# crockwell/pixelsynth

Hardware: AMD Instinct MI355X
Metric: novel-view frames/sec @256x256 (reproject+AR outpaint) (higher is better)
Workload: dtype f32

## Files before the change

### pixelsynth_amd/csrc/lmconv_grid.hip

```cpp
#include "lmconv_handle.h"

namespace pslm {

struct GemmTap {
    const float *in;
    const float *w;
    int dr, dc;
    int mask_row;
    int ld;
};

struct ItemMap {
    const int32_t *order;
    int npre;
    const int32_t *start;
    int f0;
    const int32_t *perm;
    const int2 *permq;
    const int32_t *end;
};
__device__ __forceinline__ int item_at(const ItemMap &m, int pos, int nitems)
{
    if (pos >= nitems) return -1;
    return m.perm ? m.perm[pos] : pos;
// ... 539 lines not shown
                    for (int q = 0; q < NBU; ++q) bv[h][q] = bn[h][q];
                if (j < 4) bload(j + 1, bn);
            } else {
                bload(j, bv);
            }
            __builtin_amdgcn_sched_barrier(0);
            CH_STAMP(3 * j);
            if (ALL) {
#pragma unroll
                for (int h = 0; h < NGH; ++h)
#pragma unroll
                    for (int c = 0; c < 4; ++c)
#pragma unroll
                        for (int k = 0; k < NTL; ++k)
                            acc[k] = __builtin_amdgcn_mfma_f32_16x16x4f32(av[h][a_of(k)][c], bv[h][b_of(k)][c], h == 0 && c == 0 ? zero : acc[k], 0, 0, 0);
#pragma unroll
                for (int k = 0; k < NTL; ++k) taptot[k] = j == 0 ? acc[k] : taptot[k] + acc[k];
            } else {
#pragma unroll
                for (int k = 0; k < NTL; ++k) {
                    if (!lv[k]) continue;
#pragma unroll
                    for (int h = 0; h < NGH; ++h)
#pragma unroll
                        for (int c = 0; c < 4; ++c)
                            acc[k] = __builtin_amdgcn_mfma_f32_16x16x4f32(av[h][a_of(k)][c], bv[h][b_of(k)][c], h == 0 && c == 0 ? zero : acc[k], 0, 0, 0);
                    taptot[k] = j == 0 ? acc[k] : taptot[k] + acc[k];
                }
            }
            CH_STAMP(3 * j + 1);
#pragma unroll
            for (int h = 0; h < NGH; ++h)
#pragma unroll
                for (int n = 0; n < NAU; ++n) av[h][n] = an[h][n];
#ifdef PS_WG_CHAIN_STAMPS
            __builtin_amdgcn_s_waitcnt(0x0F70);
#endif
            CH_STAMP(3 * j + 2);
            __builtin_amdgcn_sched_barrier(0);
        }
        CH_STAMP(15);
#pragma unroll
        for (int k = 0; k < NTL; ++k)
            if (lv[k]) tot[k] = tot[k] + taptot[k];
    };
    auto tap_dispatch = [&](int t, int nxt, int buf) {
        if (has5 && tiles_of(t) == (1u << TI) - 1u) tap_products(t, nxt, buf, std::integral_constant<bool, true>{});
        else tap_products(t, nxt, buf, std::integral_constant<bool, false>{});
    };
#ifndef PS_WG_TAP_SYNCTHREADS
    auto tap_barrier = [] { lds_barrier(); };
#else
    auto tap_barrier = [] { __syncthreads(); };
#endif
    int cur = next_live(-1), buf = 0;
    if (cur < ntaps) {
        stage_load(cur);
        a0_load(cur);
        stage_store(cur, 0);
    }
    __syncthreads();
    WG_STAMP(2);
    int nstamp = 3;
    (void)nstamp;
    for (int slot = 0; slot < a.nslots; ++slot) {
        for (int t = a.slot_first[slot]; t < a.slot_first[slot + 1]; ++t) {
            if (t != cur) continue;
            CH_STAMP(16);
            const int nxt = next_live(t);
            if (nxt < ntaps) stage_load(nxt);
            CH_STAMP(17);
            tap_dispatch(t, nxt, buf);
            CH_STAMP(18);
            if (DB) {
                if (nxt < ntaps) stage_store(nxt, buf ^ 1);
                CH_STAMP(19);
                tap_barrier();
                CH_STAMP(20);
                buf ^= 1;
            } else {
                tap_barrier();
                if (nxt < ntaps) stage_store(nxt, 0);
                tap_barrier();
            }
            cur = nxt;
            WG_STAMP(nstamp < 14 ? nstamp : 13);
#ifdef PS_WG_TRACE_BUILD
            ++tapno;
#endif
            ++nstamp;
        }
        if (slot == SLOT_SKIP) {
            if (fuse_post) {
                float *sY = (float *)sB;
#pragma unroll
                for (int k = 0; k < NTL; ++k)
                    if (k < NT4 || has5) *(f32x4 *)(sY + m_of(k) * YLD + NF + o_of(k) + kk * 4) = tot[k];
            } else {
#pragma unroll
                for (int k = 0; k < NTL; ++k) {
                    const int item = (k < NT4 || has5) ? sItem[m_of(k)] : -1;
                    if (item >= 0) *(f32x4 *)(a.partial + ((size_t)SLOT_SKIP * a.nitems + item) * a.Co_pad + o_of(k) + kk * 4) = tot[k];
                }
            }
        } else {
#pragma unroll
            for (int k = 0; k < NTL; ++k)
                ysum[k] = (slot == SLOT_NA ? *(const f32x4 *)(a.sum_bias + o_of(k) + kk * 4) : ysum[k]) + tot[k];
            if (slot == SLOT_NB && !fuse_post) {
#pragma unroll
                for (int k = 0; k < NTL; ++k) {
                    const int item = (k < NT4 || has5) ? sItem[m_of(k)] : -1;
                    if (item >= 0) *(f32x4 *)(a.partial + ((size_t)SLOT_NA * a.nitems + item) * a.Co_pad + o_of(k) + kk * 4) = ysum[k];
                }
            }
        }
#pragma unroll
        for (int k = 0; k < NTL; ++k) tot[k] = zero;
    }
    WG_STAMP(14);
    if (fuse_post) {
        float *sY = (float *)sB;
        Post4<POSTK, MI / GW_WAVES, GW_WAVES> post;
        post.prefetch(pa, wave, lane, sItem, sLoc);
#pragma unroll
        for (int k = 0; k < NTL; ++k)
            if (k < NT4 || has5) *(f32x4 *)(sY + m_of(k) * YLD + o_of(k) + kk * 4) = ysum[k];
        __syncthreads();
        post.run(pa, lane, sY, YLD);
    }
    WG_STAMP(15);
#ifdef PS_WG_TRACE_BUILD
    __syncthreads();
    if (a.trace_on && (y & 127) == 0 && (y >> 7) < 32 && tid < 96) g_wg_chain[KIND][y >> 7][tid / 24][tid % 24] = sChain[tid / 24][tid % 24];
#endif
    span_end();
}

#ifndef PS_WS_EXP
#define PS_WS_EXP 0
#endif
constexpr int WS_WAVES = 4, WS_THREADS = 64 * WS_WAVES, WS_MI = 16 * WS_WAVES;
constexpr int ws_occ(int kind) { return kind == GW_CONVOUT ? 2 : 3; }
template <int KIND>
__attribute__((amdgpu_waves_per_eu(ws_occ(KIND), ws_occ(KIND))))
__global__ __launch_bounds__(WS_THREADS) void k_gemm_ws(GemmArgs a, PostArgs pa)
{
    constexpr int NGH = KIND == GW_DIL ? 1 : 2, NOT = KIND == GW_CONVOUT ? 10 : 5, CO = 16 * NOT, MI = WS_MI;
    constexpr int POSTK = KIND == GW_CONVOUT ? POST_GATE : KIND == GW_CONVIN ? POST_CONVIN : POST_DIL;
    constexpr int YLD = KIND == GW_DIL ? 84 : 168;
    constexpr int HALF = 4 * CO;
    constexpr int CHUNK = NGH * HALF;
    constexpr int SVN = (CHUNK + WS_THREADS - 1) / WS_THREADS;
    constexpr int NQ = NGH * NOT;
    constexpr int NB4 = 2 * CHUNK > MI * YLD / 4 ? 2 * CHUNK : MI * YLD / 4;
    __shared__ f32x4 sA[NB4];
    __shared__ int sRow[MAX_TAPS * MI];
    __shared__ float sMv[MAX_TAPS * MI];
    __shared__ int sItem[MI], sLoc[MI];
    const int tid = threadIdx.x, wave = __builtin_amdgcn_readfirstlane(tid >> 6), lane = tid & 63, i = lane & 15, kk = lane >> 4;
    const int xcd = blockIdx.x & (N_XCD - 1), tb = blockIdx.x >> 3;
    const int y = xcd * a.tpx + tb;
    if (tb >= a.tpx || y >= a.ny) return;
    const int item0 = y * MI, ntaps = a.slot_first[a.nslots];
    const f32x4 zero = {0.0f, 0.0f, 0.0f, 0.0f};
    {
        const int pos = item0 + lane;
        int item = -1, q = 0, pat = 0x1ff;
        bool frac = true;
        if (pos < a.nitems) {
            if (a.items.permq) {
                const int2 v = a.items.permq[pos];
                item = v.x; q = v.y & 4095; pat = (v.y >> 12) & 0x1ff; frac = (v.y >> 21) & 1;
            } else {
                int fq;
                item = item_at(a.items, pos, a.nitems);
                item_loc(a.items, item, a.L, fq, q);
            }
        }
        const bool valid = item >= 0 && item_wanted(a.items, item);
        const int f = a.items.f0 + (item >= 0 ? item / a.items.npre : 0), r = q / a.W, c = q - r * a.W;
        if (wave == 0) { sItem[lane] = valid ? item : -1; sLoc[lane] = valid ? f * a.L + q : 0; }
        for (int t = wave; t < ntaps; t += WS_WAVES) {
            const GemmTap tp = a.tap[t];
            const int rr = r + tp.dr, cc = c + tp.dc;
            float mv = 0.0f;
            if (valid) {
                if (tp.mask_row < 0) mv = 1.0f;
                else if (!frac) mv = (pat >> tp.mask_row) & 1 ? 1.0f : 0.0f;
                else if (rr >= 0 && rr < a.H && cc >= 0 && cc < a.W) mv = a.mask[(size_t)f * a.mask_fstride + (size_t)tp.mask_row * a.L + q];
            }
            sRow[t * MI + lane] = mv != 0.0f ? (f * a.L + rr * a.W + cc) : -1;
            sMv[t * MI + lane] = mv;
        }
    }
    __syncthreads();
    unsigned wg_live = 0, my_live = 0;
    for (int t = 0; t < ntaps; ++t) {
        const unsigned long long b = __ballot(sRow[t * MI + lane] >= 0);
        if (b) wg_live |= 1u << t;
        if ((b >> (16 * wave)) & 0xFFFFull) my_live |= 1u << t;
    }
    if (wg_live == 0 && __ballot(sItem[lane] >= 0) == 0ull) return;
    auto next_live = [&](int t) {
        int n = t + 1;
        while (n < ntaps && !((wg_live >> n) & 1u)) ++n;
        return n;
    };
    int goff[SVN], loff[SVN];
#pragma unroll
    for (int sx = 0; sx < SVN; ++sx) {
        const int e = min(tid + WS_THREADS * sx, CHUNK - 1), h = e / HALF, r = e - h * HALF, k4 = r / CO, o = r - k4 * CO;
        goff[sx] = h * 5 * HALF + r;
        loff[sx] = h * HALF + (o >> 4) * 64 + k4 * 16 + (o & 15);
    }
    f32x4 sv[SVN];
    auto w_load = [&](int t, int j) {
        const f32x4 *w = (const f32x4 *)a.tap[t].w + j * HALF;
#pragma unroll
        for (int sx = 0; sx < SVN; ++sx) sv[sx] = w[goff[sx]];
    };
    auto w_store = [&](int buf) {
#pragma unroll
        for (int sx = 0; sx < SVN; ++sx)
            if (sx < SVN - 1 || CHUNK % WS_THREADS == 0 || tid + WS_THREADS * sx < CHUNK) sA[buf * CHUNK + loff[sx]] = sv[sx];
    };
    const float *bsrc = nullptr;
    float bmv = 0.0f;
    bool bopen = false;
    f32x4 bn[NGH];
    auto b_tap = [&](int t) {
        const int row = sRow[t * MI + wave * 16 + i];
        bmv = sMv[t * MI + wave * 16 + i];
        bopen = row >= 0;
        bsrc = (bopen ? a.tap[t].in + (size_t)row * a.tap[t].ld : (const float *)g_zero_row) + 4 * kk;
    };
    auto b_load = [&](int j) {
#pragma unroll
        for (int h = 0; h < NGH; ++h) bn[h] = *(const f32x4 *)(bsrc + 16 * (j + 5 * h));
    };
    f32x4 tot[NOT], ysum[NOT];
#pragma unroll
    for (int k = 0; k < NOT; ++k) { tot[k] = zero; ysum[k] = zero; }
    int cur = next_live(-1), buf = 0;
    if (cur < ntaps) {
        w_load(cur, 0);
        b_tap(cur);
        b_load(0);
        w_store(0);
    }
    lds_barrier();
    for (int slot = 0; slot < a.nslots; ++slot) {
        for (int t = a.slot_first[slot]; t < a.slot_first[slot + 1]; ++t) {
            if (t != cur) continue;
            const int nxt = next_live(t);
            const bool mine = (my_live >> t) & 1u;
            f32x4 taptot[NOT];
#pragma unroll
            for (int j = 0; j < 5; ++j) {
                if (!(PS_WS_EXP & 2)) { if (j < 4) w_load(t, j + 1); else w_load(nxt < ntaps ? nxt : t, 0); }
                f32x4 bv[NGH];
#pragma unroll
                for (int h = 0; h < NGH; ++h) bv[h] = bopen ? bn[h] * bmv : zero;
                if (j == 4) b_tap(nxt < ntaps ? nxt : t);
                if (!(PS_WS_EXP & 4)) b_load(j < 4 ? j + 1 : 0);
                if (mine && !(PS_WS_EXP & 1)) {
                    const f32x4 *A = sA + buf * CHUNK + lane;
                    f32x4 acc[NOT], w0 = A[0], w1 = A[64], w2 = zero, w3 = zero;
#pragma unroll
                    for (int q = 0; q < NQ; q += 2) {
                        if (q + 2 < NQ) w2 = A[((q + 2) / NOT) * HALF + ((q + 2) % NOT) * 64];
                        if (q + 3 < NQ) w3 = A[((q + 3) / NOT) * HALF + ((q + 3) % NOT) * 64];
                        __builtin_amdgcn_sched_barrier(0);
                        const int h0 = q / NOT, k0 = q % NOT, h1 = (q + 1) / NOT, k1 = (q + 1) % NOT;
#pragma unroll
                        for (int c = 0; c < 4; ++c) {
                            acc[k0] = __builtin_amdgcn_mfma_f32_16x16x4f32(w0[c], bv[h0][c], h0 == 0 && c == 0 ? zero : acc[k0], 0, 0, 0);
                            if (q + 1 < NQ)
                                acc[k1] = __builtin_amdgcn_mfma_f32_16x16x4f32(w1[c], bv[h1][c], h1 == 0 && c == 0 ? zero : acc[k1], 0, 0, 0);
                        }
                        __builtin_amdgcn_sched_barrier(0);
                        w0 = w2;
                        w1 = w3;
                    }
#pragma unroll
                    for (int k = 0; k < NOT; ++k) taptot[k] = j == 0 ? acc[k] : taptot[k] + acc[k];
                }
                if (!(PS_WS_EXP & 2)) w_store(buf ^ 1);
                if (!(PS_WS_EXP & 8)) lds_barrier();
                buf ^= 1;
            }
            if (mine && !(PS_WS_EXP & 1)) {
#pragma unroll
                for (int k = 0; k < NOT; ++k) tot[k] = tot[k] + taptot[k];
            }
            cur = nxt;
        }
        if (slot == SLOT_SKIP) {
            float *sY = (float *)sA;
#pragma unroll
            for (int k = 0; k < NOT; ++k) *(f32x4 *)(sY + (wave * 16 + i) * YLD + NF + 16 * k + kk * 4) = tot[k];
        } else {
#pragma unroll
            for (int k = 0; k < NOT; ++k) ysum[k] = (slot == SLOT_NA ? *(const f32x4 *)(a.sum_bias + 16 * k + kk * 4) : ysum[k]) + tot[k];
        }
#pragma unroll
        for (int k = 0; k < NOT; ++k) tot[k] = zero;
    }
    {
        float *sY = (float *)sA;
        Post4<POSTK, MI / WS_WAVES, WS_WAVES> post;
        post.prefetch(pa, wave, lane, sItem, sLoc);
#pragma unroll
        for (int k = 0; k < NOT; ++k) *(f32x4 *)(sY + (wave * 16 + i) * YLD + 16 * k + kk * 4) = ysum[k];
        __syncthreads();
        if (!(PS_WS_EXP & 16)) post.run(pa, lane, sY, YLD);
    }
}

struct StartsArgs {
    const int32_t *order;
    const float *mask_und, *mask_dil;
    int H, W, L, npre, F;
    int g_in[NGATED], g_out[NGATED], g_skip[NGATED], d_in[4], d_out[4];
    int32_t *starts;
    int f0;
    const int32_t *pend;
};
constexpr int STARTS_MAXL = 4096;
__global__ __launch_bounds__(1024) void k_prefix_starts(StartsArgs a)
{
    __shared__ int rank[STARTS_MAXL];
    __shared__ int s1[STARTS_MAXL];
    __shared__ int s2[STARTS_MAXL];
    __shared__ int cmin[2];
    const int f = a.f0 + blockIdx.x, t = threadIdx.x, L = a.L, npre = a.pend ? a.pend[f] : a.npre;
    const int32_t *ord = a.order + (size_t)f * L;
    for (int r = t; r < L; r += 1024) rank[ord[r]] = r;
    if (t < 2) cmin[t] = npre;
    __syncthreads();
    for (int r = t; r < L; r += 1024) {
        const int q = ord[r], y = q / a.W, x = q - y * a.W;
        int m1 = npre, m2 = npre;
        for (int tap = 0; tap < 9; ++tap) {
            if (tap == 4) continue;
            const int dy = tap / 3 - 1, dx = tap % 3 - 1;
            if (a.mask_und[((size_t)f * 9 + tap) * L + q] != 0.0f) {
                const int yy = y + dy, xx = x + dx;
                if (yy >= 0 && yy < a.H && xx >= 0 && xx < a.W) m1 = min(m1, rank[yy * a.W + xx]);
            }
            if (a.mask_dil[((size_t)f * 9 + tap) * L + q] != 0.0f) {
                const int yy = y + 2 * dy, xx = x + 2 * dx;
                if (yy >= 0 && yy < a.H && xx >= 0 && xx < a.W) m2 = min(m2, rank[yy * a.W + xx]);
            }
        }
        if (r < npre) { s1[r] = m1; s2[r] = m2; }
        else { atomicMin(&cmin[0], m1); atomicMin(&cmin[1], m2); }
    }
    __syncthreads();
    for (int off = 1; off < npre; off <<= 1) {
        int v1[STARTS_MAXL / 1024], v2[STARTS_MAXL / 1024];
#pragma unroll
        for (int k = 0; k < STARTS_MAXL / 1024; ++k) {
            const int r = t + 1024 * k;
            if (r < npre) {
                v1[k] = r + off < npre ? min(s1[r], s1[r + off]) : s1[r];
                v2[k] = r + off < npre ? min(s2[r], s2[r + off]) : s2[r];
            }
        }
        __syncthreads();
#pragma unroll
        for (int k = 0; k < STARTS_MAXL / 1024; ++k) {
            const int r = t + 1024 * k;
            if (r < npre) { s1[r] = v1[k]; s2[r] = v2[k]; }
        }
        __syncthreads();
    }
    if (t != 0) return;
    auto suf = [&](const int *s, int r0) { return r0 >= npre ? npre : min(r0, s[r0]); };
    int need[NNODE], needX[NGATED];
    for (int n = 0; n < NNODE; ++n) need[n] = npre;
    for (int g = 0; g < NGATED; ++g) { needX[g] = cmin[0]; need[a.g_in[g]] = min(need[a.g_in[g]], cmin[0]); }
    for (int d = 0; d < 4; ++d) need[a.d_in[d]] = min(need[a.d_in[d]], cmin[1]);
    const int kind[18] = {0, 0, 1, 0, 0, 1, 0, 0, 0, 0, 1, 0, 0, 0, 1, 0, 0, 0};
    const int idx[18] = {0, 1, 0, 2, 3, 1, 4, 5, 6, 7, 2, 8, 9, 10, 3, 11, 12, 13};
    int32_t *out = a.starts + f;
    for (int e = 17; e >= 0; --e) {
        if (kind[e] == 0) {
            const int g = idx[e];
            const int so = need[a.g_out[g]];
            out[(size_t)(15 + g) * a.F] = so;
            needX[g] = min(needX[g], suf(s1, so));
            need[a.g_in[g]] = min(need[a.g_in[g]], so);
            const int si = needX[g];
            out[(size_t)(1 + g) * a.F] = si;
            need[a.g_in[g]] = min(need[a.g_in[g]], suf(s1, si));
            if (a.g_skip[g] >= 0) need[a.g_skip[g]] = min(need[a.g_skip[g]], si);
        } else {
            const int d = idx[e];
            const int sd = need[a.d_out[d]];
            out[(size_t)(29 + d) * a.F] = sd;
            need[a.d_in[d]] = min(need[a.d_in[d]], suf(s2, sd));
        }
    }
    out[0] = need[0];
}

struct PermArgs {
    const int32_t *order;
    const float *mask[2];
    int H, W, L, npre, f0, nf, nparts;
    uint32_t *sorted[2];
    int32_t *cnt[2];
    int32_t *tsum[2];
    int32_t *perm[2];
    int2 *permq[2];
    const int32_t *pend;
};
constexpr int PERM_KEYS = 512;
struct PermBins { unsigned short v[PERM_KEYS]; };
constexpr PermBins make_perm_bins()
{
    PermBins t{};
    int n = 0;
    for (int pc = 9; pc >= 0; --pc)
        for (int p = 0; p < PERM_KEYS; ++p)
            if (__builtin_popcount((unsigned)p) == pc) t.v[p] = (unsigned short)n++;
    return t;
}
__device__ const PermBins g_perm_bin = make_perm_bins();
constexpr PermBins make_perm_pats()
{
    PermBins t{}, b = make_perm_bins();
    for (int p = 0; p < PERM_KEYS; ++p) t.v[b.v[p]] = (unsigned short)p;
    return t;
}
__device__ const PermBins g_perm_pat = make_perm_pats();
__device__ __forceinline__ int perm_fpp(const PermArgs &a) { return (a.nf + a.nparts - 1) / a.nparts; }
__device__ __forceinline__ size_t perm_cnt_index(const PermArgs &a, int fl, int key)
{
    const int fpp = perm_fpp(a), part = fl / fpp;
// ... 401 lines not shown
```

### pixelsynth_amd/z_buffermodel.py

```python
import math
import os
import types

import numpy as np
import torch
import torch.nn as nn

from .ar_plan import ARPlan, build_ar_plan, plan_from_reference_args
from .lmconv.layers import PONO
from .lmconv.model import TP_MIN_FRAMES, LaunchPipeline, OurPixelCNN, launch_capacity, wavefronts
from .lmconv.sample import sample
from .networks.f16x3 import checked
from .projection.z_buffer_manipulator import PtsManipulator

_PREFIX_STREAMS = {}


def rank_samples(discrim_scores, entropy_scores):
    n = len(discrim_scores)
    by_disc, by_entr = np.argsort(np.asarray(discrim_scores)), np.argsort(np.asarray(entropy_scores))
    disc_rank, entr_rank = np.empty(n, np.int64), np.empty(n, np.int64)
    disc_rank[by_disc] = np.arange(n)
    entr_rank[by_entr] = np.arange(n)
    return int(np.argmax(.5 * (n - 1 - entr_rank) + .5 * disc_rank))
# ... 25 lines not shown
        self.offset = [torch.tensor([k * V, 0], dtype=torch.int32, device=device) for k in range(depth)]
        self.order[:] = torch.arange(L, device=device, dtype=torch.int32)
        self.args = (self.codes, self.order, self.region, *self.masks)


class ZbufferModelPts(nn.Module):
    def __init__(self, opt, pts_regressor=None, vqvae=None, projector=None, encoder=None, classifier=None):
        super().__init__()
        self.opt = opt
        if pts_regressor is None and hasattr(opt, "norm_G"):
            from .networks import Unet
            extra = {"num_filters": opt.Unet_num_filters} if hasattr(opt, "Unet_num_filters") else {}
            pts_regressor = Unet(channels_in=3, channels_out=1, opt=opt, **extra)
        if projector is None and "resnet" in getattr(opt, "refine_model_type", "") and hasattr(opt, "norm_G"):
            from .networks import get_decoder
            projector = get_decoder(opt)
        self.pts_regressor = pts_regressor
        self.encoder = encoder
        if classifier is None and max(int(getattr(opt, "num_samples", 1)), 1) > 1:
            from .networks import resnet18
            classifier = resnet18(num_classes=365)
        self.classifier = classifier
        if vqvae is None and getattr(opt, "vqvae", False):
            from .vqvae2 import VQVAETop
            vqvae = VQVAETop()
        self.vqvae = vqvae
        self.projector = projector
        C = 3 if getattr(opt, "use_rgb_features", True) else 64
        self.pts_transformer = PtsManipulator(opt.W, C=C, opt=opt)
        self.num_classes = 512
        self.outpaint2 = OurPixelCNN(nr_resnet=2, nr_filters=80, input_channels=self.num_classes,
                                     nr_logistic_mix=10, kernel_size=(3, 3), max_dilation=2, weight_norm=False,
                                     feature_norm_op=lambda c: PONO(), dropout_prob=0, conv_bias=True,
                                     conv_mask_weight=False, rematerialize=False, binarize=False)
        self.args = types.SimpleNamespace(dataloader_seed=getattr(opt, "seed", 0), num_classes=self.num_classes)
        self.obs = [3, 32, 32]
        self.downsample = nn.AvgPool2d(kernel_size=8, stride=8)
        self.rotvecs = {'R': np.array([0, .6, 0]), 'L': np.array([0, -.6, 0]), 'U': np.array([-.3, 0, 0]),
                        'D': np.array([.3, 0, 0]), 'UR': np.array([-.15, .3, 0]), 'UL': np.array([-.15, -.3, 0]),
                        'DR': np.array([.15, .3, 0]), 'DL': np.array([.15, -.3, 0])}
        self.mapping = ['R', 'L', 'U', 'D', 'UL', 'UR', 'DR', 'DL']
        self.sample_batch = 32

    def eulerAnglesToRotationMatrix(self, theta):
        R_x = np.array([[1, 0, 0], [0, math.cos(theta[0]), -math.sin(theta[0])],
                        [0, math.sin(theta[0]), math.cos(theta[0])]])
        R_y = np.array([[math.cos(theta[1]), 0, math.sin(theta[1])], [0, 1, 0],
                        [-math.sin(theta[1]), 0, math.cos(theta[1])]])
        R_z = np.array([[math.cos(theta[2]), -math.sin(theta[2]), 0],
                        [math.sin(theta[2]), math.cos(theta[2]), 0], [0, 0, 1]])
        return np.dot(R_z, np.dot(R_y, R_x))

    def get_rt_from_rot(self, direction, input_RT, num=None, denom=None):
        dev = input_RT.device
        if num is None:
            num = 0
        setting = getattr(self.opt, "model_setting", "gen_img")
        if setting in ('gen_two_imgs', 'gen_scene'):
            if direction == 'S':
                new_RT = torch.zeros_like(input_RT)
                new_RT[:, :, :3] = input_RT[:, :, :3]
                new_RT[:, 3, 3] = 1
                off = torch.tensor([np.sin(2 * np.pi * num / denom), np.cos(2 * np.pi * num / denom),
                                    .4 * np.sin(2 * np.pi * (.25 + num / denom))]).to(dev)
                new_RT[0, :3, 3] = input_RT[0, :3, 3] + .35 * off
                return torch.inverse(new_RT), new_RT
            elif direction == 'C':
                rotvec = np.array([0.2 * np.cos(2 * np.pi * num / denom), 0.2 * np.sin(2 * np.pi * num / denom), 0])
            else:
                rotvec = self.rotvecs[direction] * num / denom
        else:
            rotvec = self.rotvecs[direction] * self.opt.rotation / np.linalg.norm(self.rotvecs[direction])
        mtx = torch.zeros([1, 4, 4], device=dev)
        mtx[0, 3, 3] = 1
        mtx[0, :3, :3] = torch.tensor(self.eulerAnglesToRotationMatrix(rotvec)).to(torch.float32).to(dev)
        if getattr(self.opt, "homography", False) and direction not in ('C',):
            new_RT = torch.zeros([1, 4, 4], device=dev)
            new_RT[:, :, 3] = input_RT[:, :, 3]
            new_RT[:, :3, :3] = mtx[:, :3, :3].bmm(input_RT[:, :3, :3])
        else:
            new_RT = mtx.bmm(input_RT)
        return torch.inverse(new_RT), new_RT

    def regress_depth(self, input_img, given=None):
        if self.pts_regressor is None or getattr(self.opt, "use_gt_depth", False):
            if given is None:
                raise ValueError("no depth regressor (or opt.use_gt_depth): the batch must carry the depth")
            return given
        raw = torch.sigmoid(self.pts_regressor(input_img))
        if getattr(self.opt, "use_inverse_depth", False):
            return 1. / (raw * 10 + 0.01)
        return raw * (self.opt.max_z - self.opt.min_z) + self.opt.min_z

    def get_masks_for_batch(self, output_RT, input_RTinv, background_mask, compact=False):
        plan = build_ar_plan(background_mask, self.obs[1])
        if compact:
            return plan
        b, L = plan.mask_init.shape[0], self.obs[1] * self.obs[2]
        rep = lambda m, c: m.unsqueeze(1).repeat(1, c, 1, 1).view(-1, 9, L)
        return rep(plan.mask_init, 513), rep(plan.mask_undilated, 160), rep(plan.mask_dilated, 80), plan.gen_order

    def get_combined(self, gen_fs, ar_sample, background_mask):
        b, h, w = background_mask.shape
        foreground_mask = (~background_mask).float()
        background_mask = background_mask.float()
        return gen_fs * foreground_mask.view(b, -1, h, w) + ar_sample * background_mask.view(b, -1, h, w)

    @torch.no_grad()
    def plan_views(self, fs, depth, K, K_inv, input_RT, input_RTinv, output_RT, output_RTinv):
        gen_fs, background_mask = self.pts_transformer.forward_justpts(fs, depth, K, K_inv, input_RT, input_RTinv,
                                                                      output_RT, output_RTinv)
        return dict(gen_fs=gen_fs, background_mask=background_mask, plan=build_ar_plan(background_mask, self.obs[1]))

    @staticmethod
    def adopt_planned(planned, stream):
        for t in [planned["gen_fs"], planned["background_mask"]] + planned["plan"].device_tensors():
            if t.numel():
                t.record_stream(stream)

    @torch.no_grad()
    def outpaint_planned(self, planned, codes, temperature=0.7, uniforms=None, forced=None, between=None):
        gen_fs, plan = planned["gen_fs"], planned["plan"]
        V = gen_fs.shape[0]
        L = self.obs[1] * self.obs[2]
        if codes is None:
            codes = self.vqvae.encode_codes(gen_fs)
        c32 = codes.reshape(V, L).to(torch.int32).contiguous().clone()
        eng = self.outpaint2.engine(self.obs[1], self.obs[2], V)
        if forced is None and uniforms is None:
            uniforms = torch.rand(V, L, device=gen_fs.device, dtype=torch.float32)
        nsplit = self._prefix_split(V, busy=between is not None)
        waves, pf = plan.schedule(self.PER_FRAME_PREFIX and V >= TP_MIN_FRAMES)
        args = (c32, plan.order_loc, plan.region, plan.mask_init, plan.mask_undilated, plan.mask_dilated)
        if (between is None and nsplit == 1 and not pf) or plan.first_step >= L:
            eng.ar_run(*args, temperature=temperature, uniforms=uniforms, forced=forced, first_step=plan.first_step, waves=waves)
            if between is not None:
                between()
        else:
            self._prefix_pass(eng, args, plan.first_step, 0, V, nsplit, pf, record=True)
            if between is not None:
                between()
            eng.ar_columns(*args, waves, temperature=temperature, uniforms=uniforms, forced=forced, first_step=plan.first_step)
        planned["codes"] = c32.view(V, self.obs[1], self.obs[2])
        return planned

    def _prefix_pass(self, eng, args, first_step, lo, hi, nsplit, pf, record=False):
        if nsplit == 1:
            eng.ar_prefix(*args, first_step, frame_begin=lo, frame_end=hi, **pf)
            return
        main = torch.cuda.current_stream()
        ready = torch.cuda.Event()
        ready.record(main)
        per = (hi - lo) // nsplit
        sides = self._prefix_streams(nsplit - 1, args[0].device)
        for k, side in enumerate(sides):
            side.wait_event(ready)
            with torch.cuda.stream(side):
                eng.ar_prefix(*args, first_step, frame_begin=lo + (k + 1) * per, frame_end=lo + (k + 2) * per if k + 2 < nsplit else hi, **pf)
            if record:
                for t in args + ((pf["first_steps"],) if pf else ()):
                    t.record_stream(side)
        eng.ar_prefix(*args, first_step, frame_begin=lo, frame_end=lo + per, **pf)
        for side in sides:
            main.wait_stream(side)

    PIPE_CAP = 1024
    PER_FRAME_PREFIX = True
    PIPE_DEPTH = 4
    PIPE_FRAMES = 384

    def pipe_depth(self, V):
        d = os.environ.get("PS_PIPE_DEPTH")
        if d:
            return max(2, min(8, int(d)))
        if V < TP_MIN_FRAMES:
            return self.PIPE_DEPTH
        return max(self.PIPE_DEPTH, min(8, int(round(self.PIPE_FRAMES / V))))

    def pipe_frames(self, V):
        return self.pipe_depth(V) * V

    def _pipe_buffers(self, V, device):
        st = self.__dict__.get("_pipe")
        D = self.pipe_depth(V)
        if st is not None and (st.V != V or st.device != device or st.sched.depth != D):
            if st.sched.inflight or st.sched.done:
                raise RuntimeError("outpaint_pipelined: a batch of another size is still in flight (call outpaint_flush first)")
            st = None
        if st is None:
            st = self.__dict__["_pipe"] = _PipeBuffers(V, D, self.obs[1] * self.obs[2], device)
        return st

    @torch.no_grad()
    def outpaint_pipelined(self, planned, codes, temperature=0.7, uniforms=None, between=None):
        gen_fs, plan = planned["gen_fs"], planned["plan"]
        V, G = gen_fs.shape[0], self.obs[1]
        L = G * self.obs[2]
        st = self._pipe_buffers(V, gen_fs.device)
        if codes is None:
            codes = self.vqvae.encode_codes(gen_fs)
        if uniforms is None:
            uniforms = torch.rand(V, L, device=gen_fs.device, dtype=torch.float32)
        eng = self.outpaint2.engine(G, self.obs[2], st.sched.depth * V)
        if st.sched.inflight and st.sched.inflight[0]["temperature"] != temperature:
            self._pipe_step(eng, st, drain=True)
        h = st.sched.free_slot()
        lo, hi = h * V, (h + 1) * V
        put = lambda dst, src: torch.add(src, 0, out=dst) if src.dtype == dst.dtype else dst.copy_(src)
        put(st.codes[lo:hi], codes.reshape(V, L))
        put(st.order[lo:hi], plan.order_loc)
        put(st.region[lo:hi], plan.region)
        for dst, src in zip(st.masks, (plan.mask_init, plan.mask_undilated, plan.mask_dilated)):
            put(dst[lo:hi], src.expand(V, -1, -1) if src.size(0) == 1 else src)
        put(st.uniforms[lo:hi], uniforms)
        waves, pf = plan.schedule(self.PER_FRAME_PREFIX)
        if pf:
            put(st.first_steps[lo:hi], pf["first_steps"])
            pf["first_steps"] = st.first_steps
        self._prefix_pass(eng, st.args, plan.first_step, lo, hi, self._prefix_split(V, busy=between is not None), pf)
        if between is not None:
            between()
        st.sched.admit(np.asarray(waves[1]), plan.first_step, temperature, planned=planned, slot=h,
                       cols=waves[0] + st.offset[h] if h else waves[0])
        self._pipe_step(eng, st)
        done = st.sched.pop()
        return None if done is None else done["planned"]

    def _pipe_step(self, eng, st, drain=False):
        cap = min(int(os.environ.get("PS_PIPE_CAP", self.PIPE_CAP)), self.PIPE_CAP, launch_capacity(st.V))
        for group, starts, first, temperature, finished in st.sched.step(cap, drain):
            if group:
                self._pipe_columns(eng, st, torch.cat([b["cols"][a:e] for b, a, e in group]), starts, first, temperature)
            for b in finished:
                lo = b["slot"] * st.V
                b["planned"]["codes"] = st.codes[lo:lo + st.V].clone().view(st.V, self.obs[1], self.obs[2])

    def _pipe_columns(self, eng, st, cols, ws, first, temperature):
        if len(ws) > 1 and ws[-1] > 0:
            eng.ar_columns(*st.args, (cols.contiguous(), np.ascontiguousarray(ws, np.int32)), temperature=temperature, uniforms=st.uniforms,
                           first_step=int(first))

    @torch.no_grad()
    def outpaint_flush(self):
        st = self.__dict__.get("_pipe")
        if st is None:
            return []
        if st.sched.inflight:
            self._pipe_step(self.outpaint2.engine(self.obs[1], self.obs[2], st.sched.depth * st.V), st, drain=True)
        return [b["planned"] for b in st.sched.flush()]

    def outpaint_reset(self):
        st = self.__dict__.get("_pipe")
        if st is not None:
            st.sched.reset()

    PREFIX_SPLIT_MIN_VIEWS = 64
    PREFIX_STREAMS = 2

    def _prefix_split(self, V, busy=False):
        n = int(os.environ.get("PS_PREFIX_STREAMS", self.PREFIX_STREAMS))
        if busy and "PS_PREFIX_STREAMS" not in os.environ and int(os.environ.get("GPU_MAX_HW_QUEUES", "4")) < 8:
            n = 1
        return n if n > 1 and V >= self.PREFIX_SPLIT_MIN_VIEWS and V % (8 * n) == 0 else 1

    def _prefix_streams(self, n, device):
        key = (str(device), n)
        cache = _PREFIX_STREAMS
        if key not in cache:
            skip = int(os.environ.get("PS_PREFIX_STREAM_SKIP", "0"))
            cache[("skip",) + key] = [torch.cuda.Stream(device=device) for _ in range(skip)]
            cache[key] = [torch.cuda.Stream(device=device) for _ in range(n)]
        return cache[key]

    def outpaint_views(self, fs, depth, K, K_inv, input_RT, input_RTinv, output_RT, output_RTinv, codes,
                       temperature=0.7, uniforms=None, forced=None, check=True):
        planned = self.plan_views(fs, depth, K, K_inv, input_RT, input_RTinv, output_RT, output_RTinv)
        out = self.outpaint_planned(planned, codes, temperature, uniforms, forced)
        if check:
            self.outpaint2.engine(self.obs[1], self.obs[2], fs.shape[0]).check()
        return out

    @torch.no_grad()
    def synthesize_views(self, src_imgs, view_src, K, K_inv, input_RT, input_RTinv, output_RT, output_RTinv, temperature=None,
                         uniforms=None, depths=None, check=True):
        depth_src = self.regress_depth(src_imgs, depths)
        fs_src = src_imgs if getattr(self.opt, "use_rgb_features", True) else self.encoder(src_imgs)
        planned = self.plan_views(fs_src[view_src].contiguous(), depth_src[view_src].contiguous(), K, K_inv, input_RT, input_RTinv,
                                  output_RT, output_RTinv)
        out = self.outpaint_planned(planned, None, self.opt.temperature if temperature is None else temperature, uniforms)
        if check:
            self.outpaint2.engine(self.obs[1], self.obs[2], K.shape[0]).check()
        pred = self._decode_checked(out["gen_fs"], out["background_mask"], out["codes"], check)
        return dict(PredImg=pred, FeaturesImg=out["gen_fs"], background_mask=out["background_mask"], codes=out["codes"],
                    depth=depth_src, plan=out["plan"])

    @torch.no_grad()
    def forward_image(self, batch, netD=None):
        dev = next(self.parameters()).device
        input_img = batch["images"][0].to(dev)
        cam = {k: v.to(dev) for k, v in batch["cameras"][0].items() if torch.is_tensor(v)}
        K, K_inv, input_RT, input_RTinv = cam["K"], cam["Kinv"], cam["P"], cam["Pinv"]
        paired = getattr(self.opt, "model_setting", "gen_img") == "gen_paired_img"
        if paired:
            output_img = batch["images"][-1].to(dev)
            output_RT, output_RTinv = batch["cameras"][-1]["P"].to(dev), batch["cameras"][-1]["Pinv"].to(dev)
        else:
            output_RTinv, output_RT = self.get_rt_from_rot(self.opt.direction, input_RT)
        regressed_pts = self.regress_depth(input_img, batch["depths"][0].to(dev) if "depths" in batch else None)
        fs = input_img if getattr(self.opt, "use_rgb_features", True) else self.encoder(input_img)
        gen_fs, background_mask = self.pts_transformer.forward_justpts(fs, regressed_pts, K, K_inv, input_RT,
                                                                      input_RTinv, output_RT, output_RTinv)
        outputs = {"InputImg": input_img, "PredDepthImg": regressed_pts / 5 - 1,
                   "ForegroundImg": (~background_mask).repeat(input_img.shape[0], 1, 1, 1).float(), "FeaturesImg": gen_fs}
        if paired:
            outputs["OutputImg"] = output_img
        if getattr(self.opt, "no_outpainting", False):
            outputs["PredImg"] = self._project_checked(gen_fs, None)
            return None, outputs
        if self.vqvae is not None:
            enc = getattr(self.vqvae, "encode_codes", None)
            downsampled_fs = enc(gen_fs) if enc is not None else self.vqvae.encode(gen_fs)[3]
        else:
            downsampled_fs = batch["codes"].to(dev)
        if max(int(getattr(self.opt, "num_samples", 1)), 1) > 1:
            plan = self.get_masks_for_batch(output_RT, input_RTinv, background_mask, compact=True)
            outputs["PredImg"] = self.get_best_sample(plan, downsampled_fs, background_mask, gen_fs, netD, input_img,
                                                      shard=bool(getattr(self.opt, "shard_samples", False)))
            return None, outputs
        masks_init, masks_undilated, masks_dilated, gen_order = self.get_masks_for_batch(output_RT, input_RTinv,
                                                                                         background_mask)
        autoreg_output, _ = sample(self.outpaint2, gen_order, masks_init, masks_undilated, masks_dilated,
                                   downsampled_fs, self.obs, self.args, 0, self.opt.temperature,
                                   self.downsample(background_mask.float()))
        codes = torch.argmax(autoreg_output, dim=1)
        outputs["PredCodes"] = codes
        if self.vqvae is not None:
            outputs["PredImg"] = self._decode_checked(gen_fs, background_mask, codes.to(torch.int64))
        return None, outputs

    def _entropy_score(self, gen_img):
        from PIL import Image
        raw = ((gen_img[0].reshape([256, 256, 3]).cpu().numpy() * .5 + .5) * 255).astype(np.uint8)
        im = np.asarray(Image.fromarray(raw).resize((224, 224), Image.BILINEAR), np.float32) / 255.0
        im = (im - np.array([0.485, 0.456, 0.406], np.float32)) / np.array([0.229, 0.224, 0.225], np.float32)
        x = torch.from_numpy(im).permute(2, 0, 1)[None].to(gen_img.device)
        with torch.no_grad():
            probs = torch.softmax(self.classifier(x).float().cpu(), 1).squeeze().numpy()
        probs = np.sort(probs)[::-1]
        return float(-np.sum(probs * np.log(probs)))

    def _decode_checked(self, gen_fs, background_mask, codes, check=True):
        return checked(gen_fs.device, lambda: self._project_checked(self.get_combined(gen_fs, self.vqvae.decode_code(codes), background_mask),
                                                                    background_mask), check)

    def _project_checked(self, x, *mask):
        return x if self.projector is None else checked(x.device, lambda: self.projector(x, *mask))

    @torch.no_grad()
    def get_best_sample(self, *args, uniforms=None, shard=False):
        from . import distributed as D
        if isinstance(args[0], ARPlan):
            plan, codes, background_mask, gen_fs, netD, input_img = args
        else:
            gen_order, masks, codes, background_mask, gen_fs, netD, input_img = args
            plan = plan_from_reference_args(gen_order, masks, self.downsample(background_mask.float()), gen_fs.device)
        n = max(int(getattr(self.opt, "num_samples", 1)), 1)
        if n > 1 and (netD is None or self.classifier is None):
            raise RuntimeError("num_samples > 1 ranks candidates with the discriminator (netD: pixelsynth_amd.losses.DiscriminatorLoss "
                               "or the reference's) and the scene classifier -- pass netD or use num_samples=1")
        B, G = codes.shape[0], self.obs[1]
        L = G * self.obs[2]
        dev = codes.device
        if uniforms is None:
            uniforms = torch.stack([torch.rand(B, L, generator=torch.Generator(device="cpu").manual_seed(i)) for i in range(n)]).to(dev)
        rank, world = D.world()
        mine = D.shard_views(n, rank, world) if (shard and world > 1 and n > 1) else list(range(n))
        per = max(1, min(len(mine), self.sample_batch // max(B, 1)))
        imgs, disc, entr = {}, [], []
        for s0 in range(0, len(mine), per):
            idx = mine[s0:s0 + per]
            k = len(idx)
            rep = lambda t: t.repeat((k,) + (1,) * (t.dim() - 1)).contiguous()
            waves = plan.waves
            if k > 1:
                waves = wavefronts(np.tile(plan.order_host, (k, 1)), G, self.obs[2], plan.first_step, dev)
            c = rep(codes.reshape(B, L).to(torch.int32))
            eng = self.outpaint2.engine(G, self.obs[2], k * B)
            eng.ar_run(c, rep(plan.order_loc), rep(plan.region), rep(plan.mask_init), rep(plan.mask_undilated),
                       rep(plan.mask_dilated), temperature=self.opt.temperature,
                       uniforms=uniforms[idx].reshape(k * B, L).contiguous(), first_step=plan.first_step, waves=waves)
            eng.check()
            for j, i in enumerate(idx):
                img = self._decode_checked(gen_fs, background_mask, c[j * B:(j + 1) * B].view(B, G, self.obs[2]))
                imgs[i] = img
                if n > 1:
                    disc.append(float(netD.run_discriminator_one_step(img, input_img)["D_Fake"].mean().cpu()))
                    entr.append(self._entropy_score(img))
        if n == 1:
            return imgs[0]
        if len(mine) < n:
            d_all, e_all = D.gather_scores(disc, entr, n)
            best = rank_samples(list(d_all), list(e_all))
            return D.broadcast_from(imgs.get(best), D.owner_of(best, world), gen_fs.device)
        return imgs[rank_samples(disc, entr)]

    def _scene_depth(self, img, batch):
        if self.pts_regressor is not None:
            return torch.sigmoid(self.pts_regressor(img)) * (self.opt.max_z - self.opt.min_z) + self.opt.min_z
        fn = batch.get("depth_fn")
        if fn is None:
            raise RuntimeError("forward_scene regresses depth from every generated frame: give the model a "
                               "pts_regressor or the batch a 'depth_fn' callable")
        return fn(img)

    def _scene_frame(self, st, batch, K, K_inv, in_RT, in_RTinv, out_RT, out_RTinv, netD, input_img):
        depth = self._scene_depth(st.img, batch)
        fs = st.img if getattr(self.opt, "use_rgb_features", True) else self.encoder(st.img)
        B = st.img.shape[0]
        cloud = feats = plan = uniforms = None
        if B == 1:
            gen_fs, background_mask, cloud, feats = self.pts_transformer.forward_justpts_cumulative(
                fs, depth, K, K_inv, in_RT, in_RTinv, out_RT, out_RTinv, st.cloud, st.feats, st.background, st.out_RTinv)
        else:
            gen_fs, background_mask = self._scene_step_batched(st, fs, depth, K, K_inv, in_RT, in_RTinv, out_RT, out_RTinv)
            L = self.obs[1] * self.obs[2]
# ... 141 lines not shown
```

Before: 11680.

## Split weight-staging GEMM into output-tile passes and add optional prefix stream priority

The warp-specialized GEMM kernel now processes output tiles in passes of five. The next tap's weights are loaded from global memory and stored to LDS per pass, interleaved with the MFMA work, instead of all at once. Each wave reads contiguous 64-element blocks so the LDS store index is linear, which drops the precomputed offset arrays and cuts how many staged vectors stay live in registers. The aim is lower register pressure and better overlap of weight prefetch with compute, at the cost of a different global read pattern. The Python side adds an env-controlled option to run prefix passes on high-priority side streams, optionally including the main share; it is off by default.

Result: slower. 11550 (-1.1%).

```diff
diff --git a/pixelsynth_amd/csrc/lmconv_grid.hip b/pixelsynth_amd/csrc/lmconv_grid.hip
--- a/pixelsynth_amd/csrc/lmconv_grid.hip
+++ b/pixelsynth_amd/csrc/lmconv_grid.hip
@@ -715,7 +715,9 @@
     constexpr int HALF = 4 * CO;
     constexpr int CHUNK = NGH * HALF;
     constexpr int SVN = (CHUNK + WS_THREADS - 1) / WS_THREADS;
-    constexpr int NQ = NGH * NOT;
+    constexpr int PT = 5, NPASS = NOT / PT;
+    constexpr int SH = (SVN + NPASS - 1) / NPASS;
+    constexpr int NQ = NGH * PT;
     constexpr int NB4 = 2 * CHUNK > MI * YLD / 4 ? 2 * CHUNK : MI * YLD / 4;
     __shared__ f32x4 sA[NB4];
     __shared__ int sRow[MAX_TAPS * MI];
@@ -770,23 +772,22 @@
         while (n < ntaps && !((wg_live >> n) & 1u)) ++n;
         return n;
     };
-    int goff[SVN], loff[SVN];
-#pragma unroll
-    for (int sx = 0; sx < SVN; ++sx) {
-        const int e = min(tid + WS_THREADS * sx, CHUNK - 1), h = e / HALF, r = e - h * HALF, k4 = r / CO, o = r - k4 * CO;
-        goff[sx] = h * 5 * HALF + r;
-        loff[sx] = h * HALF + (o >> 4) * 64 + k4 * 16 + (o & 15);
-    }
-    f32x4 sv[SVN];
-    auto w_load = [&](int t, int j) {
+    constexpr int NBLK = CHUNK / 64, HBLK = HALF / 64;
+    const unsigned lsrc = (unsigned)(kk * CO + i) * 16u;
+    f32x4 sv[SH];
+    auto w_load = [&](int t, int j, int p) {
         const f32x4 *w = (const f32x4 *)a.tap[t].w + j * HALF;
 #pragma unroll
-        for (int sx = 0; sx < SVN; ++sx) sv[sx] = w[goff[sx]];
-    };
-    auto w_store = [&](int buf) {
-#pragma unroll
-        for (int sx = 0; sx < SVN; ++sx)
-            if (sx < SVN - 1 || CHUNK % WS_THREADS == 0 || tid + WS_THREADS * sx < CHUNK) sA[buf * CHUNK + loff[sx]] = sv[sx];
+        for (int sx = p * SH; sx < SVN && sx < (p + 1) * SH; ++sx) {
+            const int blk = min(wave + WS_WAVES * sx, NBLK - 1);
+            const int h = blk >= HBLK ? 1 : 0;
+            sv[sx - p * SH] = *(const f32x4 *)((const char *)(w + h * 5 * HALF + (blk - h * HBLK) * 16) + lsrc);
+        }
+    };
+    auto w_store = [&](int buf, int p) {
+#pragma unroll
+        for (int sx = p * SH; sx < SVN && sx < (p + 1) * SH; ++sx)
+            if (sx < SVN - 1 || CHUNK % WS_THREADS == 0 || tid + WS_THREADS * sx < CHUNK) sA[buf * CHUNK + tid + WS_THREADS * sx] = sv[sx - p * SH];
     };
     const float *bsrc = nullptr;
     float bmv = 0.0f;
@@ -807,10 +808,10 @@
     for (int k = 0; k < NOT; ++k) { tot[k] = zero; ysum[k] = zero; }
     int cur = next_live(-1), buf = 0;
     if (cur < ntaps) {
-        w_load(cur, 0);
         b_tap(cur);
         b_load(0);
-        w_store(0);
+#pragma unroll
+        for (int p = 0; p < NPASS; ++p) { w_load(cur, 0, p); w_store(0, p); }
     }
     lds_barrier();
     for (int slot = 0; slot < a.nslots; ++slot) {
@@ -821,35 +822,39 @@
             f32x4 taptot[NOT];
 #pragma unroll
             for (int j = 0; j < 5; ++j) {
-                if (!(PS_WS_EXP & 2)) { if (j < 4) w_load(t, j + 1); else w_load(nxt < ntaps ? nxt : t, 0); }
                 f32x4 bv[NGH];
 #pragma unroll
                 for (int h = 0; h < NGH; ++h) bv[h] = bopen ? bn[h] * bmv : zero;
                 if (j == 4) b_tap(nxt < ntaps ? nxt : t);
                 if (!(PS_WS_EXP & 4)) b_load(j < 4 ? j + 1 : 0);
-                if (mine && !(PS_WS_EXP & 1)) {
-                    const f32x4 *A = sA + buf * CHUNK + lane;
-                    f32x4 acc[NOT], w0 = A[0], w1 = A[64], w2 = zero, w3 = zero;
-#pragma unroll
-                    for (int q = 0; q < NQ; q += 2) {
-                        if (q + 2 < NQ) w2 = A[((q + 2) / NOT) * HALF + ((q + 2) % NOT) * 64];
-                        if (q + 3 < NQ) w3 = A[((q + 3) / NOT) * HALF + ((q + 3) % NOT) * 64];
-                        __builtin_amdgcn_sched_barrier(0);
-                        const int h0 = q / NOT, k0 = q % NOT, h1 = (q + 1) / NOT, k1 = (q + 1) % NOT;
-#pragma unroll
-                        for (int c = 0; c < 4; ++c) {
-                            acc[k0] = __builtin_amdgcn_mfma_f32_16x16x4f32(w0[c], bv[h0][c], h0 == 0 && c == 0 ? zero : acc[k0], 0, 0, 0);
-                            if (q + 1 < NQ)
-                                acc[k1] = __builtin_amdgcn_mfma_f32_16x16x4f32(w1[c], bv[h1][c], h1 == 0 && c == 0 ? zero : acc[k1], 0, 0, 0);
+                const f32x4 *A = sA + buf * CHUNK + lane;
+#pragma unroll
+                for (int p = 0; p < NPASS; ++p) {
+                    if (!(PS_WS_EXP & 2)) { if (j < 4) w_load(t, j + 1, p); else w_load(nxt < ntaps ? nxt : t, 0, p); }
+                    if (mine && !(PS_WS_EXP & 1)) {
+                        const f32x4 *Ap = A + p * PT * 64;
+                        f32x4 acc[PT], w0 = Ap[0], w1 = Ap[64], w2 = zero, w3 = zero;
+#pragma unroll
+                        for (int q = 0; q < NQ; q += 2) {
+                            if (q + 2 < NQ) w2 = Ap[((q + 2) / PT) * HALF + ((q + 2) % PT) * 64];
+                            if (q + 3 < NQ) w3 = Ap[((q + 3) / PT) * HALF + ((q + 3) % PT) * 64];
+                            __builtin_amdgcn_sched_barrier(0);
+                            const int h0 = q / PT, k0 = q % PT, h1 = (q + 1) / PT, k1 = (q + 1) % PT;
+#pragma unroll
+                            for (int c = 0; c < 4; ++c) {
+                                acc[k0] = __builtin_amdgcn_mfma_f32_16x16x4f32(w0[c], bv[h0][c], h0 == 0 && c == 0 ? zero : acc[k0], 0, 0, 0);
+                                if (q + 1 < NQ)
+                                    acc[k1] = __builtin_amdgcn_mfma_f32_16x16x4f32(w1[c], bv[h1][c], h1 == 0 && c == 0 ? zero : acc[k1], 0, 0, 0);
+                            }
+                            __builtin_amdgcn_sched_barrier(0);
+                            w0 = w2;
+                            w1 = w3;
                         }
-                        __builtin_amdgcn_sched_barrier(0);
-                        w0 = w2;
-                        w1 = w3;
+#pragma unroll
+                        for (int k = 0; k < PT; ++k) taptot[p * PT + k] = j == 0 ? acc[k] : taptot[p * PT + k] + acc[k];
                     }
-#pragma unroll
-                    for (int k = 0; k < NOT; ++k) taptot[k] = j == 0 ? acc[k] : taptot[k] + acc[k];
+                    if (!(PS_WS_EXP & 2)) w_store(buf ^ 1, p);
                 }
-                if (!(PS_WS_EXP & 2)) w_store(buf ^ 1);
                 if (!(PS_WS_EXP & 8)) lds_barrier();
                 buf ^= 1;
             }
diff --git a/pixelsynth_amd/z_buffermodel.py b/pixelsynth_amd/z_buffermodel.py
--- a/pixelsynth_amd/z_buffermodel.py
+++ b/pixelsynth_amd/z_buffermodel.py
@@ -201,15 +201,17 @@
         ready = torch.cuda.Event()
         ready.record(main)
         per = (hi - lo) // nsplit
-        sides = self._prefix_streams(nsplit - 1, args[0].device)
-        for k, side in enumerate(sides):
+        own = self._prefix_stream_priority() == 2
+        sides = self._prefix_streams(nsplit if own else nsplit - 1, args[0].device)
+        for k, side in enumerate(sides, 0 if own else 1):
             side.wait_event(ready)
             with torch.cuda.stream(side):
-                eng.ar_prefix(*args, first_step, frame_begin=lo + (k + 1) * per, frame_end=lo + (k + 2) * per if k + 2 < nsplit else hi, **pf)
+                eng.ar_prefix(*args, first_step, frame_begin=lo + k * per, frame_end=lo + (k + 1) * per if k + 1 < nsplit else hi, **pf)
             if record:
                 for t in args + ((pf["first_steps"],) if pf else ()):
                     t.record_stream(side)
-        eng.ar_prefix(*args, first_step, frame_begin=lo, frame_end=lo + per, **pf)
+        if not own:
+            eng.ar_prefix(*args, first_step, frame_begin=lo, frame_end=lo + per, **pf)
         for side in sides:
             main.wait_stream(side)
 
@@ -318,8 +320,14 @@
         if key not in cache:
             skip = int(os.environ.get("PS_PREFIX_STREAM_SKIP", "0"))
             cache[("skip",) + key] = [torch.cuda.Stream(device=device) for _ in range(skip)]
-            cache[key] = [torch.cuda.Stream(device=device) for _ in range(n)]
+            prio = min(torch.cuda.Stream.priority_range()) if self._prefix_stream_priority() else 0
+            cache[key] = [torch.cuda.Stream(device=device, priority=prio) for _ in range(n)]
         return cache[key]
+
+    PREFIX_STREAM_PRIORITY = 0
+
+    def _prefix_stream_priority(self):
+        return int(os.environ.get("PS_PREFIX_STREAM_PRIORITY", self.PREFIX_STREAM_PRIORITY))
 
     def outpaint_views(self, fs, depth, K, K_inv, input_RT, input_RTinv, output_RT, output_RTinv, codes,
                        temperature=0.7, uniforms=None, forced=None, check=True):
```
